# chechaohp/gan-ode

Measured on AMD Instinct MI355X. Metric: generated videos/sec (16-frame clips), higher is better.
Workload: dtype f32

## Files before the change

### gan-ode_amd/_lib.py

```python
from __future__ import annotations

import ctypes as C
import os

_HERE = os.path.dirname(os.path.abspath(__file__))
LIB_PATH = os.path.join(_HERE, "lib", "libgode.so")

i32, i64, f32, ptr = C.c_int32, C.c_int64, C.c_float, C.c_void_p
cint, u32, u64 = C.c_int, C.c_uint32, C.c_uint64

ACT_NONE, ACT_RELU, ACT_LRELU, ACT_TANH_OUT = 0, 1, 2, 3
EPI_RAW, EPI_TANH = 0, 1
FPROP, DGRAD = 0, 1
OP_IGEMM, OP_WGRAD, OP_BN_FINALIZE, OP_BN_BWD, OP_ODE_FWD, OP_ODE_BWD, OP_BCE, OP_ADAM, OP_PACK = range(1, 10)
OP_ODERNN_FWD, OP_ODERNN_BWD, OP_BN_APPLY, OP_COL2IM = 10, 11, 12, 13
OP_SDE_FWD, OP_SDE_BWD = 14, 15
OP_CDE_FWD, OP_CDE_BWD = 16, 17
OP_WGAN = 18
OP_GRU_FWD, OP_GRU_BWD = 19, 20
OP_DNOISE = 21
OP_CATEG, OP_CE = 22, 23
OP_CHSTATS, OP_CBN_EMBED, OP_CBN_EMBED_BWD, OP_CBN_APPLY, OP_CBN_BWD, OP_GRES_OUT, OP_GRES_OUT_BWD, OP_SN_FWD, OP_SN_BWD = range(24, 33)
REC_ADAM_NOISE = -1
ODE_NPARAM = 2672
# ... 111 lines not shown

class CdeFwdOp(_Op):
    _fields_ = [("p", CdeParams), ("x", ptr), ("tslope", ptr), ("content", ptr), ("sel_t", ptr), ("z", ptr),
                ("states", ptr), ("sched", ptr), ("counts", ptr), ("sync", ptr), ("N", i32), ("T", i32),
                ("S_cap", i32), ("zcols", i32), ("rtol", f32), ("atol", f32)]
    KIND, FN = OP_CDE_FWD, "gode_cde_fwd"


class CdeBwdOp(_Op):
    _fields_ = [("p", CdeParams), ("x", ptr), ("tslope", ptr), ("sel_t", ptr), ("states", ptr), ("sched", ptr),
                ("counts", ptr), ("gz", ptr), ("work", ptr), ("grads", ptr), ("N", i32), ("T", i32), ("S_cap", i32),
                ("accumulate", i32), ("zcols", i32), ("pad_", i32)]
    KIND, FN = OP_CDE_BWD, "gode_cde_bwd"


class GruParams(C.Structure):
    _fields_ = [(n, ptr) for n in "Wih Whh bih bhh".split()]


class GruFwdOp(_Op):
    _fields_ = [("p", GruParams), ("noise", ptr), ("content", ptr), ("sel_t", ptr), ("z", ptr), ("hs", ptr), ("N", i32),
                ("T", i32), ("zcols", i32), ("pad_", i32)]
    KIND, FN = OP_GRU_FWD, "gode_gru_fwd"


class GruBwdOp(_Op):
    _fields_ = [("p", GruParams), ("noise", ptr), ("hs", ptr), ("sel_t", ptr), ("gz", ptr), ("work", ptr), ("grads", ptr),
                ("N", i32), ("T", i32), ("accumulate", i32), ("zcols", i32)]
    KIND, FN = OP_GRU_BWD, "gode_gru_bwd"


class BnApplyOp(_Op):
    _fields_ = [("y", ptr), ("out", ptr), ("scale", ptr), ("shift", ptr), ("M", i64), ("C", i32), ("act", i32),
                ("M0", i64)]
    KIND, FN = OP_BN_APPLY, "gode_bn_apply"


class DnoiseOp(_Op):
    _fields_ = [("x", ptr), ("out", ptr), ("scale", ptr), ("shift", ptr), ("call_dev", ptr), ("M", i64), ("C", i32),
                ("act", i32), ("M0", i64), ("e_off", i64), ("xs", i64 * 5), ("N", i32), ("D", i32), ("H", i32), ("W", i32),
                ("seed", i64), ("stream", i32), ("layer", i32), ("call", i32), ("sigma", f32)]
    KIND, FN = OP_DNOISE, "gode_dnoise"


class Col2imOp(_Op):
    _fields_ = [("cols", ptr), ("out", ptr)] + [(n, i32) for n in "N Hi Wi Ho Wo C kh kw sh sw ph pw epilogue pad_ Di Do kd sd pd pad2_".split()]
    KIND, FN = OP_COL2IM, "gode_col2im"


class BceOp(_Op):
    _fields_ = [("logits", ptr), ("grad", ptr), ("loss", ptr), ("n", i64), ("target", f32), ("gscale", f32),
                ("accumulate", i32), ("stride", i32)]
    KIND, FN = OP_BCE, "gode_bce_logits"


class CategOp(_Op):
    _fields_ = [("cls", ptr), ("z", ptr), ("labels_out", ptr), ("n_traj", i32), ("rows_per", i32), ("C", i32),
                ("zcols", i32), ("col0", i32), ("pad_", i32)]
    KIND, FN = OP_CATEG, "gode_categ_onehot"


class CeOp(_Op):
    _fields_ = [("logits", ptr), ("labels", ptr), ("grad", ptr), ("loss", ptr), ("B", i32), ("n_lab", i32), ("C", i32),
                ("ld", i32), ("gld", i32), ("gscale", f32), ("accumulate", i32), ("rows_per_label", i32)]
    KIND, FN = OP_CE, "gode_ce_logits"


# ... 50 lines not shown
    KIND, FN = OP_SN_FWD, "gode_sn_fwd"


class SnBwdOp(_Op):
    _fields_ = [("G", ptr), ("wbar", ptr), ("u", ptr), ("v", ptr), ("sigma", ptr), ("dwbar", ptr), ("work", ptr), ("h", i32),
                ("w", i32)]
    KIND, FN = OP_SN_BWD, "gode_sn_bwd"


class AdamNoiseTensor(C.Structure):
    _fields_ = [("p", ptr), ("g", ptr), ("m", ptr), ("v", ptr), ("n", i64), ("noise_off", i64)]


class AdamOp(_Op):
    _fields_ = [("p", ptr), ("g", ptr), ("m", ptr), ("v", ptr), ("n", i64), ("lr", f32), ("beta1", f32),
                ("beta2", f32), ("eps", f32), ("weight_decay", f32), ("gscale", f32), ("step", i32), ("pad_", i32)]
    KIND, FN = OP_ADAM, "gode_adam_l2"


class PackOp(C.Structure):
    _fields_ = [("g", ConvGeom), ("dir", i32), ("co_canon", i32), ("w", ptr), ("wpack", ptr), ("co_perm", ptr)]
    KIND = OP_PACK


_OPS = _Op.__subclasses__()
_STRUCTS = {0: ConvGeom, REC_ADAM_NOISE: AdamNoiseTensor, OP_PACK: PackOp, **{st.KIND: st for st in _OPS}}

_PROTOS = {
    "gode_igemm_stats_rows": ([ptr], cint),
    "gode_igemm_stats_rows0": ([ptr], cint),
    "gode_igemm_stats_segments": ([ptr, i32, ptr], cint),
    "gode_igemm_model_cycles": ([ptr], C.c_double),
    "gode_igemm_work_size": ([ptr], i64),
    "gode_pack_size": ([ptr, cint], i64),
    "gode_pack_weights": ([ptr, cint, ptr, ptr, ptr, i32, ptr], cint),
    "gode_wgrad_work_size": ([ptr], i64),
    "gode_wgrad_auto_splits": ([ptr], cint),
    "gode_bn_bwd_work_size": ([i64, i32], i64),
    "gode_ode_bwd_work_size": ([i32], i64),
    "gode_odernn_bwd_work_size": ([i32], i64),
    "gode_odernn_sync_size": ([i32], i64),
    "gode_sde_bwd_work_size": ([i32], i64),
    "gode_cde_sync_size": ([i32], i64),
    "gode_cde_state_size": ([i32, i32], i64),
    "gode_cde_bwd_work_size": ([i32], i64),
    "gode_gru_bwd_work_size": ([i32], i64),
    "gode_ode_fwd_multi": ([ptr, i32, ptr], cint),
    "gode_ode_bwd_multi": ([ptr, i32, ptr], cint),
    "gode_odernn_fwd_multi": ([ptr, i32, ptr], cint),
    "gode_odernn_bwd_multi": ([ptr, i32, ptr], cint),
    "gode_gru_fwd_multi": ([ptr, i32, ptr], cint),
    "gode_gru_bwd_multi": ([ptr, i32, ptr], cint),
    "gode_chstats_rows": ([i64], cint),
    "gode_cbn_bwd_work_size": ([i32, i32, i32, i32], i64),
    "gode_gres_out_bwd_work_size": ([i32, i32, i32, i32, i32, i32], i64),
    "gode_scale": ([ptr, ptr, i64, f32, cint, ptr], cint),
    "gode_adam_multi": ([ptr, i32, i64, f32, f32, f32, f32, f32, f32, i32, ptr], cint),
    "gode_adam_multi_dev": ([ptr, i32, i64, f32, f32, f32, f32, f32, ptr, ptr], cint),
    "gode_adam_noise_multi": ([ptr, i32, i64, f32, f32, f32, f32, f32, f32, i32, u64, u32, u32, f32, ptr], cint),
    "gode_adam_noise_multi_dev": ([ptr, i32, i64, f32, f32, f32, f32, f32, ptr, u64, u32, f32, ptr], cint),
    "gode_param_noise": ([ptr, i64, u64, u32, u32, i64, f32, i32, ptr], cint),
    "gode_dnoise_normals": ([ptr, i64, u64, u32, u32, u32, i64, i32, ptr], cint),
    "gode_ode_step_chunks": ([ptr, i64], i64),
    "gode_ode_step": ([ptr, i32, i64, i32, f32, f32, f32, f32, f32, ptr, ptr], cint),
    "gode_axpy_multi": ([ptr, i32, i64, f32, ptr, ptr, f32, ptr, ptr, ptr], cint),
    "gode_run": ([ptr, ptr, i32, ptr], cint),
# ... 82 lines not shown
```

### gan-ode_amd/csrc/elementwise.hip

```cpp
#include "common.h"
#include "philox.h"

__global__ void __launch_bounds__(256) bn_finalize_kernel(const gode_bn_finalize_op a) {
  const int c = blockIdx.x, tid = threadIdx.x;
  __shared__ double red[2][256];
  if (a.training) {
    const int reps = a.ncols / a.C;
    const int ngroups = a.groups == 2 ? 2 : 1;
    for (int gi = 0; gi < ngroups; ++gi) {
      const int grp = ngroups == 2 ? (a.order ? 1 - gi : gi) : 0;
      double s1 = 0.0, s2 = 0.0;
      const int nseg = (ngroups == 2 && !a.stats1) ? (a.nseg > 0 ? a.nseg : 1) : 1;
      for (int sg = 0; sg < nseg; ++sg) {
        int r_lo, r_hi;
        if (ngroups == 1 || a.stats1) { r_lo = 0; r_hi = (grp == 1 && a.stats1) ? a.rows1 : a.rows; }
        else if (a.nseg > 0) { r_lo = grp == 0 ? a.seg[3 * sg] : a.seg[3 * sg + 1]; r_hi = grp == 0 ? a.seg[3 * sg + 1] : a.seg[3 * sg + 2]; }
        else { r_lo = grp == 0 ? 0 : a.rows0; r_hi = grp == 0 ? a.rows0 : a.rows; }
        const float* st = (grp == 1 && a.stats1) ? a.stats1 : a.stats;
        const int stride = (grp == 1 && a.stats1) ? a.rows1 : a.rows;
        const int nr = r_hi - r_lo;
        const int64_t items = (int64_t)nr * reps;
        for (int64_t i = tid; i < items; i += 256) {
          const int rep = (int)(i / nr); const int r = r_lo + (int)(i - (int64_t)rep * nr);
          const int64_t o = (int64_t)(rep * a.C + c) * stride + r;
          s1 += (double)st[o];
          s2 += (double)st[(int64_t)a.ncols * stride + o];
        }
      }
      __syncthreads();
      red[0][tid] = s1; red[1][tid] = s2;
      __syncthreads();
      for (int s = 128; s > 0; s >>= 1) {
        if (tid < s) { red[0][tid] += red[0][tid + s]; red[1][tid] += red[1][tid + s]; }
        __syncthreads();
      }
      if (tid == 0) {
        const double n = (double)((grp == 1 && a.count1 > 0) ? a.count1 : a.count);
        const double mean = red[0][0] / n;
        double var = red[1][0] / n - mean * mean;
        if (var < 0.0) var = 0.0;
        const float invstd = (float)(1.0 / sqrt(var + (double)a.eps));
        const float g = a.gamma ? a.gamma[c] : 1.f, b = a.beta ? a.beta[c] : 0.f;
        const float sc = g * invstd;
        const int o = grp * a.C + c;
        a.mean[o] = (float)mean; a.invstd[o] = invstd;
        a.scale[o] = sc; a.shift[o] = b - (float)mean * sc;
        if (a.running_mean) {
          const double unbiased = n > 1.0 ? var * n / (n - 1.0) : var;
          a.running_mean[c] = (1.f - a.momentum) * a.running_mean[c] + a.momentum * (float)mean;
          a.running_var[c] = (1.f - a.momentum) * a.running_var[c] + a.momentum * (float)unbiased;
        }
        if (c == 0 && a.num_batches_tracked) *a.num_batches_tracked += 1;
      }
    }
  } else if (tid == 0) {
    const float invstd = 1.f / sqrtf(a.running_var[c] + a.eps);
    const float g = a.gamma ? a.gamma[c] : 1.f, b = a.beta ? a.beta[c] : 0.f;
    const float sc = g * invstd;
    const int ngroups = a.groups == 2 ? 2 : 1;
    for (int grp = 0; grp < ngroups; ++grp) {
      const int o = grp * a.C + c;
      if (a.mean) a.mean[o] = a.running_mean[c];
      if (a.invstd) a.invstd[o] = invstd;
      a.scale[o] = sc; a.shift[o] = b - a.running_mean[c] * sc;
    }
  }
}

extern "C" int gode_bn_finalize(const gode_bn_finalize_op* op, void* stream) {
  if (!op || op->C <= 0 || !op->scale || !op->shift) return GODE_E_ARG;
  if (op->training) {
    if (!op->stats || !op->mean || !op->invstd || op->ncols % op->C != 0 || op->count <= 0) return GODE_E_ARG;
    if (op->stats1 && (op->groups != 2 || op->rows1 <= 0 || op->rows <= 0)) return GODE_E_ARG;
    if (op->groups == 2 && !op->stats1 && op->nseg == 0 && (op->rows0 <= 0 || op->rows0 >= op->rows)) return GODE_E_ARG;
    if (op->groups == 2 && (op->nseg < 0 || op->nseg > 8)) return GODE_E_ARG;
    for (int i = 0; op->groups == 2 && i < op->nseg; ++i)
      if (!(0 <= op->seg[3 * i] && op->seg[3 * i] <= op->seg[3 * i + 1] && op->seg[3 * i + 1] <= op->seg[3 * i + 2] && op->seg[3 * i + 2] <= op->rows)) return GODE_E_ARG;
  } else if (!op->running_mean || !op->running_var) return GODE_E_ARG;
  hipLaunchKernelGGL(bn_finalize_kernel, dim3(op->C), dim3(256), 0, (hipStream_t)stream, *op);
  GODE_LAUNCH_CHECK();
  return 0;
}

__global__ void __launch_bounds__(256) bn_apply_kernel(const gode_bn_apply_op a) {
  const int64_t n4 = a.M * a.C / 4;
  const float neg = a.act == GODE_ACT_RELU ? 0.f : (a.act == GODE_ACT_LRELU ? 0.2f : 1.f);
  for (int64_t i = (int64_t)blockIdx.x * 256 + threadIdx.x; i < n4; i += (int64_t)gridDim.x * 256) {
    const int c = (int)((i * 4) % a.C) + ((a.M0 > 0 && i * 4 >= a.M0 * a.C) ? a.C : 0);
    f32x4 v = *reinterpret_cast<const f32x4*>(a.y + i * 4);
    f32x4 sc = {1.f, 1.f, 1.f, 1.f}, sh = {0.f, 0.f, 0.f, 0.f};
    if (a.scale) { sc = *reinterpret_cast<const f32x4*>(a.scale + c); sh = *reinterpret_cast<const f32x4*>(a.shift + c); }
#pragma unroll
    for (int e = 0; e < 4; ++e) { const float t = v[e] * sc[e] + sh[e]; v[e] = fmaxf(t, t * neg); }
    *reinterpret_cast<f32x4*>(a.out + i * 4) = v;
  }
}

extern "C" int gode_bn_apply(const gode_bn_apply_op* op, void* stream) {
  if (!op || !op->y || !op->out || op->M <= 0 || op->C <= 0 || op->C % 4 != 0) return GODE_E_ARG;
  if ((op->scale == nullptr) != (op->shift == nullptr)) return GODE_E_ARG;
  int64_t b = (op->M * op->C / 4 + 255) / 256;
  hipLaunchKernelGGL(bn_apply_kernel, dim3((int)(b > 8192 ? 8192 : (b < 1 ? 1 : b))), dim3(256), 0, (hipStream_t)stream, *op);
  GODE_LAUNCH_CHECK();
  return 0;
}

__global__ void __launch_bounds__(256) col2im_kernel(const gode_col2im_op a) {
  const int64_t total = (int64_t)a.N * a.Ho * a.Wo;
  const int KC = a.kh * a.kw * a.C;
  for (int64_t i = (int64_t)blockIdx.x * 256 + threadIdx.x; i < total; i += (int64_t)gridDim.x * 256) {
    const int ow = (int)(i % a.Wo); const int64_t t = i / a.Wo;
    const int oh = (int)(t % a.Ho), n = (int)(t / a.Ho);
    float acc[4] = {0.f, 0.f, 0.f, 0.f};
    for (int kh = (oh + a.ph) % a.sh; kh < a.kh; kh += a.sh) {
      const int ih = (oh + a.ph - kh) / a.sh;
      if (oh + a.ph - kh < 0 || ih >= a.Hi) continue;
      for (int kw = (ow + a.pw) % a.sw; kw < a.kw; kw += a.sw) {
        const int iw = (ow + a.pw - kw) / a.sw;
        if (ow + a.pw - kw < 0 || iw >= a.Wi) continue;
        const float* src = a.cols + ((int64_t)(n * a.Hi + ih) * a.Wi + iw) * KC + (kh * a.kw + kw) * a.C;
        for (int c = 0; c < a.C; ++c) acc[c] += src[c];
      }
    }
    float* dst = a.out + i * a.C;
    for (int c = 0; c < a.C; ++c) dst[c] = a.epilogue == GODE_EPI_TANH ? tanhf(acc[c]) : acc[c];
  }
}

__global__ void __launch_bounds__(256) col2im_rows_kernel(const gode_col2im_op a, int R, int nq) {
  extern __shared__ __attribute__((aligned(16))) float c2i_lds[];
  const int KC = a.kh * a.kw * a.C, rowlen = a.Wi * KC;
  const int q = blockIdx.x % nq, n = blockIdx.x / nq;
// ... 575 lines not shown
```

### gan-ode_amd/csrc/igemm.hip

```cpp
#include <stdlib.h>
#include "common.h"
#include "conv_geom.h"

int gode_launch_conv_patch_fprop(const gode_igemm_op* op, const int64_t* gs, hipStream_t st);

struct IgemmArgs {
  IgemmGeom G;
  const float* src;
  const float* w;
  float* out;
  const float* scale;
  const float* shift;
  float* stats;
  int32_t gsN, gsD, gsH, gsW, gsC;
  int32_t act, epilogue;
  int32_t MB, NB, xcd_mode;
  int32_t tapskip, dmajor;
  int32_t stagger;
  int32_t ksplit, slabs_per_split;
  float* work;
  int32_t out_numel;
  int32_t stats_rows;
  uint32_t src_bytes, w_bytes;
};
// ... 729 lines not shown
      const float s = (part[0][threadIdx.x] + part[1][threadIdx.x]) + (part[2][threadIdx.x] + part[3][threadIdx.x]);
      a.out[oo + threadIdx.x] = a.epilogue == GODE_EPI_TANH ? tanhf(s) : s;
    }
  }
}

#define PW_MAXW 4096
struct PwArgs { IgemmArgs a; FastDiv dMw[GODE_MAX_PHASES], dMh[GODE_MAX_PHASES], dMd[GODE_MAX_PHASES]; int32_t lpp; };

template <bool ONE_TAP>
__global__ void __launch_bounds__(256) conv_pointwise_kernel(const PwArgs d) {
  const IgemmArgs& a = d.a;
  const int ph = blockIdx.y;
  const PhaseGeom& P = a.G.ph[ph];
  const int Ncols = a.G.Ncols, Cg = a.G.Cg;
  __shared__ __attribute__((aligned(16))) float wl[ONE_TAP ? 4 : PW_MAXW];
  if (!ONE_TAP) {
    for (int i = threadIdx.x; i < Ncols * P.Kp; i += 256) wl[i] = a.w[P.w_off + i];
    __syncthreads();
  }
  const int lane = threadIdx.x & 63, lpp = d.lpp, ppw = 64 / lpp;
  const int sub = lane / lpp, ch = (lane - sub * lpp) * 4;
  const float neg = a.act == GODE_ACT_RELU ? 0.f : (a.act == GODE_ACT_LRELU ? 0.2f : 1.f);
  f32x4 sc = {1.f, 1.f, 1.f, 1.f}, sh = {0.f, 0.f, 0.f, 0.f};
  if (a.scale) { sc = *reinterpret_cast<const f32x4*>(a.scale + ch); sh = *reinterpret_cast<const f32x4*>(a.shift + ch); }
  const int ntap = ONE_TAP ? 1 : P.Td * P.Th * P.Tw;
  f32x4 w1[4];
  if (ONE_TAP) {
#pragma unroll
    for (int n = 0; n < 4; ++n)
      w1[n] = n < Ncols ? *reinterpret_cast<const f32x4*>(a.w + P.w_off + (int64_t)n * P.Kp + ch) : f32x4{0.f, 0.f, 0.f, 0.f};
  }
  const int64_t wave_id = (int64_t)blockIdx.x * 4 + (threadIdx.x >> 6), nwaves = (int64_t)gridDim.x * 4;
  for (int64_t m0 = wave_id * ppw; m0 < P.M; m0 += nwaves * ppw) {
    const int m = (int)m0 + sub;
    const bool live = m < P.M;
    const uint32_t mm = live ? (uint32_t)m : 0u;
    const uint32_t t1 = fdiv(mm, d.dMw[ph]), qw = mm - t1 * P.Mw;
    const uint32_t t2 = fdiv(t1, d.dMh[ph]), qh = t1 - t2 * P.Mh;
    const uint32_t img = fdiv(t2, d.dMd[ph]), qd = t2 - img * P.Md;
    const int bd = (int)qd * a.G.Sd + P.Od, bh = (int)qh * a.G.Sh + P.Oh, bw = (int)qw * a.G.Sw + P.Ow;
    const int base = (int)img * a.gsN;
    float acc[4] = {0.f, 0.f, 0.f, 0.f};
    int jd = 0, jh = 0, jw = 0;
    for (int t = 0; t < ntap; ++t) {
      const int id = bd + a.G.J * jd, ih = bh + a.G.J * jh, iw = bw + a.G.J * jw;
      const bool ok = live && (unsigned)id < (unsigned)a.G.Gd && (unsigned)ih < (unsigned)a.G.Gh && (unsigned)iw < (unsigned)a.G.Gw;
      if (ok) {
        f32x4 v = *reinterpret_cast<const f32x4*>(a.src + base + id * a.gsD + ih * a.gsH + iw * a.gsW + ch);
#pragma unroll
        for (int e = 0; e < 4; ++e) { const float u = v[e] * sc[e] + sh[e]; v[e] = fmaxf(u, u * neg); }
        const float* wk = wl + t * Cg + ch;
#pragma unroll
        for (int n = 0; n < 4; ++n)
          if (ONE_TAP || n < Ncols) {
            const f32x4 w = ONE_TAP ? w1[n] : *reinterpret_cast<const f32x4*>(wk + n * P.Kp);
            acc[n] += v[0] * w[0] + v[1] * w[1] + v[2] * w[2] + v[3] * w[3];
          }
      }
      if (++jw == P.Tw) { jw = 0; if (++jh == P.Th) { jh = 0; ++jd; } }
    }
    for (int o = lpp >> 1; o > 0; o >>= 1) {
#pragma unroll
      for (int n = 0; n < 4; ++n) acc[n] += __shfl_xor(acc[n], o);
    }
    if (live && ch == 0) {
// ... 625 lines not shown
```

### gan-ode_amd/engine.py

```python
from __future__ import annotations

import ctypes as C
from dataclasses import dataclass
from typing import List, Optional, Sequence

import numpy as np
import torch

from . import _lib as L


def make_geom(N, Ci, Co, xi, yo, k, s, p) -> L.ConvGeom:
    return L.ConvGeom(N, Ci, Co, xi[0], xi[1], xi[2], yo[0], yo[1], yo[2], k[0], k[1], k[2], s[0], s[1], s[2],
                      p[0], p[1], p[2])


def conv_out(i, k, s, p):
    return (i + 2 * p - k) // s + 1


def dptr(t: Optional[torch.Tensor]):
    return None if t is None else t.data_ptr()


# ... 31 lines not shown
    beta: Optional[torch.Tensor] = None
    running_mean: Optional[torch.Tensor] = None
    running_var: Optional[torch.Tensor] = None
    num_batches_tracked: Optional[torch.Tensor] = None


def _contig_strides(dims):
    n, d, h, w, c = dims
    return (d * h * w * c, h * w * c, w * c, c, 1)


class ConvStack:

    def __init__(self, specs: Sequence[LayerSpec], params: Sequence[LayerParams], device, owns_input: bool,
                 momentum=0.1, eps=1e-5, pack_cache: Optional[dict] = None, groups: int = 1, split_images: int = 0,
                 split_order: int = 0, two_lane_backward: bool = False):
        self.specs, self.params, self.device = list(specs), list(params), device
        self.groups = groups
        self.two_lane = bool(two_lane_backward)
        self._lane_stream = None
        self.split, self.split_order = int(split_images), int(split_order)
        if self.split and (groups != 1 or not owns_input or not (0 < self.split < specs[0].geom.N)):
            raise ValueError("split ConvStack: plan-owned input, one launch group, 0 < split_images < N")
        self._G2 = groups == 2 or self.split > 0
        self._last_parts = False
        if groups not in (1, 2) or (groups == 2 and (owns_input or specs[0].fwd_dir != L.FPROP or specs[0].has_bn
                                                     or specs[0].geom.N % 2)):
            raise ValueError("grouped ConvStack: two groups, Conv stack, caller-owned input, no BatchNorm on layer 0")
        self.nl = len(specs)
        self.noisy = any(s.noise for s in specs)
        if self.noisy and (owns_input or self.split):
            raise ValueError("instance noise: caller-owned input, no split stack")
        self.momentum, self.eps = momentum, eps
        self.busy = False
        self.generation = 0
        self._fwd_training = True
        self.pack_cache = pack_cache if pack_cache is not None else {}
        lib = L.lib()
        f32 = dict(dtype=torch.float32, device=device)
        self.x_in = torch.zeros(specs[0].in_dims(), **f32) if owns_input else None
        self.x0n = torch.empty(specs[0].in_dims(), **f32) if specs[0].noise else None
        self.y = [torch.empty(s.out_dims(), **f32) for s in specs[:-1]]
        self.a = [torch.empty(s.out_dims(), **f32) if self._materialize(l) else None for l, s in enumerate(specs[:-1])]
        self.out_dims = specs[-1].out_dims()
        self.wpack_f, self.wpack_b = [], [None] * self.nl
        self.stats, self.stat_rows = [], []
        self.mean, self.invstd, self.scale, self.shift = [], [], [], []
        self._two_f, self._two_b, self._rows_ab = {}, {}, {}
        for l, s in enumerate(specs):
            n = lib.gode_pack_size(C.byref(s.geom), s.fwd_dir)
            if n <= 0:
                raise RuntimeError(f"bad geometry for pack ({n})")
            self.wpack_f.append(self._shared_pack(l, s.fwd_dir, n))
            C_out = s.out_dims()[4]
            two = self._two_f[l] = bool(self.split) and 0 < l < self.nl - 1 and self._two_launches(s.geom, s.fwd_dir)
            if s.has_bn:
                probe = L.IgemmOp(g=s.geom, dir=s.fwd_dir, tile=0, groups=groups)
                if two:
                    ra, rb = (lib.gode_igemm_stats_rows(C.byref(L.IgemmOp(g=self._part_geom(s.geom, n), dir=s.fwd_dir, tile=0)))
                              for n in (self.split, s.geom.N - self.split))
                    rows = ra + rb if ra > 0 and rb > 0 else -1
                    self._rows_ab[l] = (ra, rb)
                else:
                    rows = lib.gode_igemm_stats_rows(C.byref(probe))
                if rows <= 0:
                    raise RuntimeError(f"layer {l}: no partial-statistics layout for this geometry ({rows})")
# ... 228 lines not shown
                    raise RuntimeError("a one-layer stack cannot use the GEMM + col2im head")
                continue
            want_stats = s.has_bn and training
            if self._last_parts and l == self.nl - 1:
                per_in, per_out, Cs = int(np.prod(s.in_dims()[1:])), int(np.prod(s.out_dims()[1:])), sc.numel() // 2
                pair = []
                for n, img0, k in ((self.split, 0, 0), (s.geom.N - self.split, self.split, 1)):
                    pair.append(L.IgemmOp(g=self._part_geom(s.geom, n), dir=s.fwd_dir, act=act, epilogue=s.epilogue, tile=0,
                                          src=src.data_ptr() + 4 * img0 * per_in, wpack=dptr(self.wpack_f[l]), out=None,
                                          scale=sc.data_ptr() + 4 * Cs * k, shift=sh.data_ptr() + 4 * Cs * k))
                ops += pair
                patch["last"], patch["last2"] = pair[0], (pair[1], 4 * self.split * per_out)
                continue
            if self._two_f.get(l):
                ra = self._rows_ab[l][0] if s.has_bn else 0
                per_in, per_out = int(np.prod(s.in_dims()[1:])), int(np.prod(s.out_dims()[1:]))
                for n, img0, st_off in ((self.split, 0, 0), (s.geom.N - self.split, self.split, ra * 2 * self._ncols(s))):
                    ops.append(L.IgemmOp(g=self._part_geom(s.geom, n), dir=s.fwd_dir, act=act, epilogue=s.epilogue, tile=0,
                                         src=src.data_ptr() + 4 * img0 * per_in, wpack=dptr(self.wpack_f[l]),
                                         out=self.y[l].data_ptr() + 4 * img0 * per_out, scale=dptr(sc), shift=dptr(sh),
                                         stats=self.stats[l].data_ptr() + 4 * st_off if want_stats else None, groups=0))
                op = None
            else:
                op = L.IgemmOp(g=s.geom, dir=s.fwd_dir, act=act, epilogue=s.epilogue, tile=0, src=dptr(src),
                               wpack=dptr(self.wpack_f[l]), out=dptr(self.y[l]) if l < self.nl - 1 else None,
                               scale=dptr(sc), shift=dptr(sh),
                               stats=dptr(self.stats[l]) if want_stats else None,
                               groups=2 if (G2 and s.has_bn) else 0)
                ops.append(op)
            if l == 0:
                patch["first"] = op
            if l == self.nl - 1:
                patch["last"] = op
            if s.has_bn:
                rows0 = lib.gode_igemm_stats_rows0(C.byref(op)) if G2 else 0
                fin = L.BnFinalizeOp(stats=dptr(self.stats[l]), rows=self.stat_rows[l], ncols=self._ncols(s),
                                     C=s.out_dims()[4], count=self._count(l) // self.groups, gamma=dptr(p.gamma),
                                     beta=dptr(p.beta), running_mean=dptr(p.running_mean),
                                     running_var=dptr(p.running_var),
                                     num_batches_tracked=dptr(p.num_batches_tracked), mean=dptr(self.mean[l]),
                                     invstd=dptr(self.invstd[l]), scale=dptr(self.scale[l]),
                                     shift=dptr(self.shift[l]), momentum=self.momentum, eps=self.eps,
                                     training=1 if training else 0, groups=self.groups if G2 else 0, rows0=rows0)
                if self.split:
                    per_img = self._count(l) // s.geom.N
                    fin.groups, fin.order = 2, self.split_order
                    fin.count, fin.count1 = per_img * self.split, per_img * (s.geom.N - self.split)
                    if self._two_f.get(l):
                        ra, rb = self._rows_ab[l]
                        fin.rows, fin.rows1 = ra, rb
                        fin.stats1 = self.stats[l].data_ptr() + 4 * ra * 2 * self._ncols(s)
                    else:
                        nseg, seg = self._segs[l]
                        fin.nseg = nseg
                        for k in range(3 * nseg):
                            fin.seg[k] = seg[k]
                ops.append(fin)
            if l < self.nl - 1 and self.a[l] is not None:
                d = s.out_dims()
                M = d[0] * d[1] * d[2] * d[3]
                M0 = M // 2 if (G2 and s.has_bn) else ((M // d[0]) * self.split if (self.split and s.has_bn) else 0)
                if self.specs[l + 1].noise:
                    ops.append(self._noise_op(noise, l, dptr(self.scale[l]), dptr(self.shift[l]), M // 2 if G2 else 0))
                    continue
                ops.append(L.BnApplyOp(y=dptr(self.y[l]), out=dptr(self.a[l]), scale=dptr(self.scale[l]),
                                       shift=dptr(self.shift[l]), M=M, C=d[4], act=s.act, M0=M0))
        patch["packs"] = packs
        self._attach_work([op for op in ops if isinstance(op, L.IgemmOp)])
        return L.Program(ops), patch

    def _noise_op(self, noise, l, scale, shift, M0):
        d = self.specs[l].out_dims()
        op = L.DnoiseOp(x=dptr(self.y[l]), out=dptr(self.a[l]), scale=scale, shift=shift, M=d[0] * d[1] * d[2] * d[3],
                        C=d[4], act=self.specs[l].act, M0=M0, layer=l + 1)
        noise.append((op, d[1] * d[2] * d[3] * d[4], 0, None))
        return op

    @staticmethod
    def _patch_noise(patch, noise, inputs):
        seed = int(noise["seed"]) & 0xFFFFFFFFFFFFFFFF
        seed = seed - (1 << 64) if seed >= 1 << 63 else seed
        dev = noise.get("call_dev")
        base = 0 if dev else int(noise["call"])
        for op, per, add, k in patch["noise"]:
            op.seed, op.stream, op.sigma = seed, int(noise["stream"]), float(noise["sigma"])
            c = (base + add) & 0xFFFFFFFF
            op.call_dev, op.call = dev, c - (1 << 32) if c >= 1 << 31 else c
            op.e_off = int(noise.get("sample_offset", 0)) * per
            if k is not None:
                x, xs = inputs[k]
                op.x = x.data_ptr()
                for i in range(5):
                    op.xs[i] = int(xs[i])

    def forward(self, training: bool, x: Optional[torch.Tensor] = None, x_strides=None, pre_ops_program=None,
                x2: Optional[torch.Tensor] = None, x2_strides=None, noise=None):
        self._refresh()
        if training not in self._fwd:
            self._fwd[training] = self._build_fwd(training)
        prog, patch = self._fwd[training]
        if self.noisy:
            if noise is None:
# ... 285 lines not shown
```

### include/gode.h

```cpp
#ifndef GODE_H
#define GODE_H
#include <stdint.h>
#ifdef __cplusplus
extern "C" {
#endif

#define GODE_VERSION 105

enum { GODE_OK = 0, GODE_E_ARG = -1, GODE_E_SHAPE = -2, GODE_E_KIND = -3 };
enum { GODE_ACT_NONE = 0, GODE_ACT_RELU = 1, GODE_ACT_LRELU = 2,
       GODE_ACT_TANH_OUT = 3  };
enum { GODE_EPI_RAW = 0, GODE_EPI_TANH = 1 };
enum { GODE_FPROP = 0, GODE_DGRAD = 1 };

typedef struct gode_conv_geom {
  int32_t N, Ci, Co;
  int32_t Di, Hi, Wi;
  int32_t Do, Ho, Wo;
  int32_t kd, kh, kw;
  int32_t sd, sh, sw;
  int32_t pd, ph, pw;
} gode_conv_geom;

typedef struct gode_igemm_op {
// ... 20 lines not shown
                      int32_t co_canon, void* stream);

typedef struct gode_wgrad_op {
  gode_conv_geom g;
  int32_t act, xform_on_y, splits, accumulate;
  const float* x;
  const float* y;
  const float* scale;
  const float* shift;
  float* work;
  float* dw;
  const int32_t* co_perm; int64_t co_canon;
  int64_t xs[5];
} gode_wgrad_op;
int gode_wgrad(const gode_wgrad_op* op, void* stream);
int64_t gode_wgrad_work_size(const gode_wgrad_op* op);
int gode_wgrad_auto_splits(const gode_conv_geom* g);

typedef struct gode_bn_finalize_op {
  const float* stats; int32_t rows, ncols, C; int64_t count;
  const float* gamma; const float* beta;
  float* running_mean; float* running_var; int64_t* num_batches_tracked;
  float* mean; float* invstd; float* scale; float* shift;
  float momentum, eps; int32_t training, pad_;
  int32_t groups, rows0;
  int32_t nseg, order; int64_t count1; int32_t seg[24];
  const float* stats1; int32_t rows1, pad3_;
} gode_bn_finalize_op;
int gode_bn_finalize(const gode_bn_finalize_op* op, void* stream);

typedef struct gode_bn_apply_op {
  const float* y; float* out; const float* scale; const float* shift; int64_t M; int32_t C, act;
  int64_t M0;
} gode_bn_apply_op;
int gode_bn_apply(const gode_bn_apply_op* op, void* stream);

typedef struct gode_col2im_op {
  const float* cols; float* out;
  int32_t N, Hi, Wi, Ho, Wo, C, kh, kw, sh, sw, ph, pw;
  int32_t epilogue, pad_;
  int32_t Di, Do, kd, sd, pd, pad2_;
} gode_col2im_op;
int gode_col2im(const gode_col2im_op* op, void* stream);

typedef struct gode_bn_bwd_op {
  float* g; const float* y; int64_t M; int32_t C, act;
  const float* gamma; const float* mean; const float* invstd; const float* scale; const float* shift;
  float* dgamma; float* dbeta; float* work; int32_t accumulate, eval_mode;
  const float* gin;
  int32_t groups, pad2_;
  int64_t M0;
  const float* r1_s; const float* r1_w; int32_t r1_H, r1_W, r1_h, r1_wd, r1_off, pad3_;
} gode_bn_bwd_op;
int gode_bn_bwd(const gode_bn_bwd_op* op, void* stream);
int64_t gode_bn_bwd_work_size(int64_t M, int32_t C);

typedef struct gode_ode_params {
  const float* Wa; const float* ba; const float* Wb; const float* bb;
  const float* W1; const float* b1; const float* W2; const float* b2;
} gode_ode_params;
typedef struct gode_ode_fwd_op {
  gode_ode_params p;
  const float* x; const float* content; const float* dt; const int32_t* sel_t;
  float* z; float* traj; int32_t N, T, substeps, prenet;
  int32_t zcols, G;
  const float* grid_dt; const int32_t* emit_at; const float* emit_w;
  int32_t method, pad2_; float rtol, atol; const float* tout; int32_t* nsteps;
  int32_t* sync;
// ... 285 lines not shown
```

Measured before the change: 35290.

## Fold BN finalize into BN apply kernel and unroll one-tap pointwise path

Adds a fused bn_apply_fold kernel. Each block recomputes the per-channel batch-norm statistics for a slice of channels, then applies scale, shift and activation to a chunk of rows. This removes a separate finalize launch and its dependency. The price is redundant re-reading of the stats across row chunks, and a cost model decides when the fold is used. A separate change adds a 4-way unrolled one-tap path in the igemm pointwise kernel to batch its loads.

New measurement: 34050. 3.5% lower.

```diff
diff --git a/gan-ode_amd/_lib.py b/gan-ode_amd/_lib.py
--- a/gan-ode_amd/_lib.py
+++ b/gan-ode_amd/_lib.py
@@ -167,7 +167,7 @@
 
 class BnApplyOp(_Op):
     _fields_ = [("y", ptr), ("out", ptr), ("scale", ptr), ("shift", ptr), ("M", i64), ("C", i32), ("act", i32),
-                ("M0", i64)]
+                ("M0", i64), ("fold", i32), ("pad_", i32), ("fin", BnFinalizeOp)]
     KIND, FN = OP_BN_APPLY, "gode_bn_apply"
 
 
@@ -284,6 +284,7 @@
     "gode_igemm_stats_segments": ([ptr, i32, ptr], cint),
     "gode_igemm_model_cycles": ([ptr], C.c_double),
     "gode_igemm_work_size": ([ptr], i64),
+    "gode_bn_apply_fold_pays": ([i32, i32, i32, i64], cint),
     "gode_pack_size": ([ptr, cint], i64),
     "gode_pack_weights": ([ptr, cint, ptr, ptr, ptr, i32, ptr], cint),
     "gode_wgrad_work_size": ([ptr], i64),
diff --git a/gan-ode_amd/csrc/elementwise.hip b/gan-ode_amd/csrc/elementwise.hip
--- a/gan-ode_amd/csrc/elementwise.hip
+++ b/gan-ode_amd/csrc/elementwise.hip
@@ -1,32 +1,87 @@
 #include "common.h"
 #include "philox.h"
+
+
+__device__ __forceinline__ int bn_ngroups(const gode_bn_finalize_op& a) { return a.groups == 2 ? 2 : 1; }
+__device__ __forceinline__ int bn_group(const gode_bn_finalize_op& a, int gi) { return a.groups == 2 ? (a.order ? 1 - gi : gi) : 0; }
+
+struct BnSeg { const float* st; int64_t plane; int stride, r_lo, nr, reps; int64_t items; };
+__device__ __forceinline__ int64_t bn_item(const gode_bn_finalize_op& a, const BnSeg& s, int c, int64_t i) {
+  const int rep = (int)(i / s.nr); const int r = s.r_lo + (int)(i - (int64_t)rep * s.nr);
+  return (int64_t)(rep * a.C + c) * s.stride + r;
+}
+template <class F>
+__device__ __forceinline__ void bn_walk(const gode_bn_finalize_op& a, int grp, F&& f) {
+  const int ngroups = bn_ngroups(a);
+  const int nseg = (ngroups == 2 && !a.stats1) ? (a.nseg > 0 ? a.nseg : 1) : 1;
+  for (int sg = 0; sg < nseg; ++sg) {
+    int r_lo, r_hi;
+    if (ngroups == 1 || a.stats1) { r_lo = 0; r_hi = (grp == 1 && a.stats1) ? a.rows1 : a.rows; }
+    else if (a.nseg > 0) { r_lo = grp == 0 ? a.seg[3 * sg] : a.seg[3 * sg + 1]; r_hi = grp == 0 ? a.seg[3 * sg + 1] : a.seg[3 * sg + 2]; }
+    else { r_lo = grp == 0 ? 0 : a.rows0; r_hi = grp == 0 ? a.rows0 : a.rows; }
+    BnSeg s;
+    s.st = (grp == 1 && a.stats1) ? a.stats1 : a.stats;
+    s.stride = (grp == 1 && a.stats1) ? a.rows1 : a.rows;
+    s.plane = (int64_t)a.ncols * s.stride;
+    s.r_lo = r_lo; s.nr = r_hi - r_lo; s.reps = a.ncols / a.C;
+    s.items = (int64_t)s.nr * s.reps;
+    f(s);
+  }
+}
+__device__ __forceinline__ void bn_channel_train(const gode_bn_finalize_op& a, int c, int grp, double s1, double s2, bool write,
+                                                 float& sc_out, float& sh_out) {
+  const double n = (double)((grp == 1 && a.count1 > 0) ? a.count1 : a.count);
+  const double mean = s1 / n;
+  double var = s2 / n - mean * mean;
+  if (var < 0.0) var = 0.0;
+  const float invstd = (float)(1.0 / sqrt(var + (double)a.eps));
+  const float g = a.gamma ? a.gamma[c] : 1.f, b = a.beta ? a.beta[c] : 0.f;
+  const float sc = g * invstd;
+  const float sh = b - (float)mean * sc;
+  sc_out = sc; sh_out = sh;
+  if (write) {
+    const int o = grp * a.C + c;
+    a.mean[o] = (float)mean; a.invstd[o] = invstd;
+    a.scale[o] = sc; a.shift[o] = sh;
+    if (a.running_mean) {
+      const double unbiased = n > 1.0 ? var * n / (n - 1.0) : var;
+      a.running_mean[c] = (1.f - a.momentum) * a.running_mean[c] + a.momentum * (float)mean;
+      a.running_var[c] = (1.f - a.momentum) * a.running_var[c] + a.momentum * (float)unbiased;
+    }
+    if (c == 0 && a.num_batches_tracked) *a.num_batches_tracked += 1;
+  }
+}
+__device__ __forceinline__ void bn_channel_eval(const gode_bn_finalize_op& a, int c, bool write, float& sc_out, float& sh_out) {
+  const float invstd = 1.f / sqrtf(a.running_var[c] + a.eps);
+  const float g = a.gamma ? a.gamma[c] : 1.f, b = a.beta ? a.beta[c] : 0.f;
+  const float sc = g * invstd;
+  const float sh = b - a.running_mean[c] * sc;
+  sc_out = sc; sh_out = sh;
+  if (write) {
+    for (int grp = 0; grp < bn_ngroups(a); ++grp) {
+      const int o = grp * a.C + c;
+      if (a.mean) a.mean[o] = a.running_mean[c];
+      if (a.invstd) a.invstd[o] = invstd;
+      a.scale[o] = sc; a.shift[o] = sh;
+    }
+  }
+}
 
 __global__ void __launch_bounds__(256) bn_finalize_kernel(const gode_bn_finalize_op a) {
   const int c = blockIdx.x, tid = threadIdx.x;
   __shared__ double red[2][256];
+  float sc, sh;
   if (a.training) {
-    const int reps = a.ncols / a.C;
-    const int ngroups = a.groups == 2 ? 2 : 1;
-    for (int gi = 0; gi < ngroups; ++gi) {
-      const int grp = ngroups == 2 ? (a.order ? 1 - gi : gi) : 0;
+    for (int gi = 0; gi < bn_ngroups(a); ++gi) {
+      const int grp = bn_group(a, gi);
       double s1 = 0.0, s2 = 0.0;
-      const int nseg = (ngroups == 2 && !a.stats1) ? (a.nseg > 0 ? a.nseg : 1) : 1;
-      for (int sg = 0; sg < nseg; ++sg) {
-        int r_lo, r_hi;
-        if (ngroups == 1 || a.stats1) { r_lo = 0; r_hi = (grp == 1 && a.stats1) ? a.rows1 : a.rows; }
-        else if (a.nseg > 0) { r_lo = grp == 0 ? a.seg[3 * sg] : a.seg[3 * sg + 1]; r_hi = grp == 0 ? a.seg[3 * sg + 1] : a.seg[3 * sg + 2]; }
-        else { r_lo = grp == 0 ? 0 : a.rows0; r_hi = grp == 0 ? a.rows0 : a.rows; }
-        const float* st = (grp == 1 && a.stats1) ? a.stats1 : a.stats;
-        const int stride = (grp == 1 && a.stats1) ? a.rows1 : a.rows;
-        const int nr = r_hi - r_lo;
-        const int64_t items = (int64_t)nr * reps;
-        for (int64_t i = tid; i < items; i += 256) {
-          const int rep = (int)(i / nr); const int r = r_lo + (int)(i - (int64_t)rep * nr);
-          const int64_t o = (int64_t)(rep * a.C + c) * stride + r;
-          s1 += (double)st[o];
-          s2 += (double)st[(int64_t)a.ncols * stride + o];
+      bn_walk(a, grp, [&](const BnSeg& s) {
+        for (int64_t i = tid; i < s.items; i += 256) {
+          const int64_t o = bn_item(a, s, c, i);
+          s1 += (double)s.st[o];
+          s2 += (double)s.st[s.plane + o];
         }
-      }
+      });
       __syncthreads();
       red[0][tid] = s1; red[1][tid] = s2;
       __syncthreads();
@@ -34,40 +89,12 @@
         if (tid < s) { red[0][tid] += red[0][tid + s]; red[1][tid] += red[1][tid + s]; }
         __syncthreads();
       }
-      if (tid == 0) {
-        const double n = (double)((grp == 1 && a.count1 > 0) ? a.count1 : a.count);
-        const double mean = red[0][0] / n;
-        double var = red[1][0] / n - mean * mean;
-        if (var < 0.0) var = 0.0;
-        const float invstd = (float)(1.0 / sqrt(var + (double)a.eps));
-        const float g = a.gamma ? a.gamma[c] : 1.f, b = a.beta ? a.beta[c] : 0.f;
-        const float sc = g * invstd;
-        const int o = grp * a.C + c;
-        a.mean[o] = (float)mean; a.invstd[o] = invstd;
-        a.scale[o] = sc; a.shift[o] = b - (float)mean * sc;
-        if (a.running_mean) {
-          const double unbiased = n > 1.0 ? var * n / (n - 1.0) : var;
-          a.running_mean[c] = (1.f - a.momentum) * a.running_mean[c] + a.momentum * (float)mean;
-          a.running_var[c] = (1.f - a.momentum) * a.running_var[c] + a.momentum * (float)unbiased;
-        }
-        if (c == 0 && a.num_batches_tracked) *a.num_batches_tracked += 1;
-      }
-    }
-  } else if (tid == 0) {
-    const float invstd = 1.f / sqrtf(a.running_var[c] + a.eps);
-    const float g = a.gamma ? a.gamma[c] : 1.f, b = a.beta ? a.beta[c] : 0.f;
-    const float sc = g * invstd;
-    const int ngroups = a.groups == 2 ? 2 : 1;
-    for (int grp = 0; grp < ngroups; ++grp) {
-      const int o = grp * a.C + c;
-      if (a.mean) a.mean[o] = a.running_mean[c];
-      if (a.invstd) a.invstd[o] = invstd;
-      a.scale[o] = sc; a.shift[o] = b - a.running_mean[c] * sc;
-    }
-  }
-}
-
-extern "C" int gode_bn_finalize(const gode_bn_finalize_op* op, void* stream) {
+      if (tid == 0) bn_channel_train(a, c, grp, red[0][0], red[1][0], true, sc, sh);
+    }
+  } else if (tid == 0) bn_channel_eval(a, c, true, sc, sh);
+}
+
+static int bn_finalize_check(const gode_bn_finalize_op* op) {
   if (!op || op->C <= 0 || !op->scale || !op->shift) return GODE_E_ARG;
   if (op->training) {
     if (!op->stats || !op->mean || !op->invstd || op->ncols % op->C != 0 || op->count <= 0) return GODE_E_ARG;
@@ -77,27 +104,178 @@
     for (int i = 0; op->groups == 2 && i < op->nseg; ++i)
       if (!(0 <= op->seg[3 * i] && op->seg[3 * i] <= op->seg[3 * i + 1] && op->seg[3 * i + 1] <= op->seg[3 * i + 2] && op->seg[3 * i + 2] <= op->rows)) return GODE_E_ARG;
   } else if (!op->running_mean || !op->running_var) return GODE_E_ARG;
+  return 0;
+}
+
+extern "C" int gode_bn_finalize(const gode_bn_finalize_op* op, void* stream) {
+  const int rc = bn_finalize_check(op);
+  if (rc) return rc;
   hipLaunchKernelGGL(bn_finalize_kernel, dim3(op->C), dim3(256), 0, (hipStream_t)stream, *op);
   GODE_LAUNCH_CHECK();
   return 0;
 }
+
+__device__ __forceinline__ f32x4 bn_act4(f32x4 v, const f32x4& sc, const f32x4& sh, float neg) {
+#pragma unroll
+  for (int e = 0; e < 4; ++e) { const float t = v[e] * sc[e] + sh[e]; v[e] = fmaxf(t, t * neg); }
+  return v;
+}
+__device__ __forceinline__ float bn_neg_slope(int act) { return act == GODE_ACT_RELU ? 0.f : (act == GODE_ACT_LRELU ? 0.2f : 1.f); }
 
 __global__ void __launch_bounds__(256) bn_apply_kernel(const gode_bn_apply_op a) {
   const int64_t n4 = a.M * a.C / 4;
-  const float neg = a.act == GODE_ACT_RELU ? 0.f : (a.act == GODE_ACT_LRELU ? 0.2f : 1.f);
+  const float neg = bn_neg_slope(a.act);
   for (int64_t i = (int64_t)blockIdx.x * 256 + threadIdx.x; i < n4; i += (int64_t)gridDim.x * 256) {
     const int c = (int)((i * 4) % a.C) + ((a.M0 > 0 && i * 4 >= a.M0 * a.C) ? a.C : 0);
-    f32x4 v = *reinterpret_cast<const f32x4*>(a.y + i * 4);
+    const f32x4 v = *reinterpret_cast<const f32x4*>(a.y + i * 4);
     f32x4 sc = {1.f, 1.f, 1.f, 1.f}, sh = {0.f, 0.f, 0.f, 0.f};
     if (a.scale) { sc = *reinterpret_cast<const f32x4*>(a.scale + c); sh = *reinterpret_cast<const f32x4*>(a.shift + c); }
-#pragma unroll
-    for (int e = 0; e < 4; ++e) { const float t = v[e] * sc[e] + sh[e]; v[e] = fmaxf(t, t * neg); }
-    *reinterpret_cast<f32x4*>(a.out + i * 4) = v;
-  }
+    *reinterpret_cast<f32x4*>(a.out + i * 4) = bn_act4(v, sc, sh, neg);
+  }
+}
+
+#ifndef BN_FOLD_SLICE
+#define BN_FOLD_SLICE 32
+#endif
+#define BN_FOLD_WGS 512
+struct BnFoldGrid { int32_t nslices, nchunks; int64_t rows_per_chunk; };
+
+__device__ __forceinline__ double bn_fold_sum(const gode_bn_finalize_op& f, int grp, int which, int c, int j) {
+  double acc[32];
+#pragma unroll
+  for (int k = 0; k < 32; ++k) acc[k] = 0.0;
+  bn_walk(f, grp, [&](const BnSeg& s) {
+    const float* st = s.st + (int64_t)which * s.plane;
+    int64_t base = 0;
+    for (; base + 256 <= s.items; base += 256) {
+      float v[32];
+#pragma unroll
+      for (int k = 0; k < 32; ++k) {
+        const int64_t i = base + 8 * k + j;
+        v[k] = st[s.reps == 1 ? (int64_t)c * s.stride + s.r_lo + i : bn_item(f, s, c, i)];
+      }
+#pragma unroll
+      for (int k = 0; k < 32; ++k) acc[k] += (double)v[k];
+    }
+    if (base < s.items) {
+#pragma unroll
+      for (int kb = 0; kb < 32; kb += 8) {
+        if (base + 8 * kb < s.items) {
+          float v[8];
+#pragma unroll
+          for (int k = 0; k < 8; ++k) {
+            const int64_t i = base + 8 * (kb + k) + j;
+            const bool ok = i < s.items;
+            const int64_t o = s.reps == 1 ? (int64_t)c * s.stride + s.r_lo + (ok ? i : 0) : bn_item(f, s, c, ok ? i : 0);
+            const float x = st[o];
+            v[k] = ok ? x : 0.f;
+          }
+#pragma unroll
+          for (int k = 0; k < 8; ++k) acc[kb + k] += (double)v[k];
+        }
+      }
+    }
+  });
+#pragma unroll
+  for (int s = 16; s > 0; s >>= 1) {
+#pragma unroll
+    for (int k = 0; k < 16; ++k)
+      if (k < s) acc[k] += acc[k + s];
+  }
+  double x = acc[0];
+#pragma unroll
+  for (int s = 4; s > 0; s >>= 1) x += __shfl_xor(x, s);
+  return x;
+}
+
+__global__ void __launch_bounds__(256) bn_apply_fold_kernel(const gode_bn_apply_op a, const BnFoldGrid g) {
+  const gode_bn_finalize_op& f = a.fin;
+  __shared__ __attribute__((aligned(16))) float ssc[2][BN_FOLD_SLICE], ssh[2][BN_FOLD_SLICE];
+  const int tid = threadIdx.x;
+  const int sl = (int)(blockIdx.x % g.nslices), chunk = (int)(blockIdx.x / g.nslices);
+  const int c0 = sl * BN_FOLD_SLICE;
+  const bool writer = chunk == 0;
+  for (int cb = 0; cb < BN_FOLD_SLICE; cb += 32) {
+    const int cl = cb + (tid >> 3), c = c0 + cl, j = tid & 7;
+    const bool live = c < f.C;
+    const int cc = live ? c : 0;
+    float sc = 1.f, sh = 0.f;
+    if (f.training) {
+      for (int gi = 0; gi < bn_ngroups(f); ++gi) {
+        const int grp = bn_group(f, gi);
+        const double s1 = bn_fold_sum(f, grp, 0, cc, j);
+        const double s2 = bn_fold_sum(f, grp, 1, cc, j);
+        if (live) {
+          bn_channel_train(f, c, grp, s1, s2, writer && j == 0, sc, sh);
+          if (j == 0) { ssc[grp][cl] = sc; ssh[grp][cl] = sh; }
+        }
+      }
+    } else if (live && j == 0) {
+      bn_channel_eval(f, c, writer, sc, sh);
+      ssc[0][cl] = sc; ssh[0][cl] = sh; ssc[1][cl] = sc; ssh[1][cl] = sh;
+    }
+  }
+  __syncthreads();
+  constexpr int LPR = BN_FOLD_SLICE / 4, RPI = 256 / LPR;
+  const int q = tid % LPR, c = c0 + q * 4;
+  if (c >= a.C) return;
+  const float neg = bn_neg_slope(a.act);
+  const f32x4 sc0 = *reinterpret_cast<const f32x4*>(&ssc[0][q * 4]), sh0 = *reinterpret_cast<const f32x4*>(&ssh[0][q * 4]);
+  const f32x4 sc1 = *reinterpret_cast<const f32x4*>(&ssc[1][q * 4]), sh1 = *reinterpret_cast<const f32x4*>(&ssh[1][q * 4]);
+  const int64_t m_lo = chunk * g.rows_per_chunk;
+  const int64_t m_hi = m_lo + g.rows_per_chunk < a.M ? m_lo + g.rows_per_chunk : a.M;
+  for (int64_t m = m_lo + tid / LPR; m < m_hi; m += 4 * RPI) {
+    f32x4 v[4];
+#pragma unroll
+    for (int u = 0; u < 4; ++u)
+      if (m + u * RPI < m_hi) v[u] = *reinterpret_cast<const f32x4*>(a.y + (m + u * RPI) * a.C + c);
+#pragma unroll
+    for (int u = 0; u < 4; ++u)
+      if (m + u * RPI < m_hi) {
+        const bool second = a.M0 > 0 && m + u * RPI >= a.M0;
+        *reinterpret_cast<f32x4*>(a.out + (m + u * RPI) * a.C + c) = bn_act4(v[u], second ? sc1 : sc0, second ? sh1 : sh0, neg);
+      }
+  }
+}
+
+static int bn_fold_grid(const gode_bn_apply_op* op, BnFoldGrid* g) {
+  const int64_t nsl = (op->C + BN_FOLD_SLICE - 1) / BN_FOLD_SLICE;
+  int64_t nch = (BN_FOLD_WGS + nsl - 1) / nsl;
+  const int64_t rpi = 256 / (BN_FOLD_SLICE / 4);
+  if (nch > (op->M + rpi - 1) / rpi) nch = (op->M + rpi - 1) / rpi;
+  if (nch < 1) nch = 1;
+  g->nslices = (int32_t)nsl;
+  g->rows_per_chunk = (op->M + nch - 1) / nch;
+  g->nchunks = (int32_t)((op->M + g->rows_per_chunk - 1) / g->rows_per_chunk);
+  return nsl * g->nchunks < (1ll << 31) ? 0 : GODE_E_SHAPE;
+}
+
+#define BN_FOLD_MAX_REREAD 0.5
+extern "C" int gode_bn_apply_fold_pays(int32_t rows, int32_t ncols, int32_t C, int64_t M) {
+  if (rows <= 0 || C <= 0 || C % 4 != 0 || ncols <= 0 || ncols % C != 0 || M <= 0) return GODE_E_ARG;
+  gode_bn_apply_op op = {};
+  op.C = C; op.M = M;
+  BnFoldGrid g;
+  if (bn_fold_grid(&op, &g)) return 0;
+  const double reread = (double)g.nslices * g.nchunks * BN_FOLD_SLICE * ((double)rows * (ncols / C)) * 8.0;
+  const double pass = (double)M * C * 8.0;
+  return reread <= BN_FOLD_MAX_REREAD * pass ? 1 : 0;
 }
 
 extern "C" int gode_bn_apply(const gode_bn_apply_op* op, void* stream) {
   if (!op || !op->y || !op->out || op->M <= 0 || op->C <= 0 || op->C % 4 != 0) return GODE_E_ARG;
+  if (op->fold) {
+    const int rc = bn_finalize_check(&op->fin);
+    if (rc) return rc;
+    if (op->fin.C != op->C) return GODE_E_ARG;
+    if (op->fin.training && (int64_t)(op->fin.rows > op->fin.rows1 ? op->fin.rows : op->fin.rows1) * (op->fin.ncols / op->fin.C) >= (1ll << 31))
+      return GODE_E_SHAPE;
+    BnFoldGrid g;
+    if (bn_fold_grid(op, &g)) return GODE_E_SHAPE;
+    hipLaunchKernelGGL(bn_apply_fold_kernel, dim3(g.nslices * g.nchunks), dim3(256), 0, (hipStream_t)stream, *op, g);
+    GODE_LAUNCH_CHECK();
+    return 0;
+  }
   if ((op->scale == nullptr) != (op->shift == nullptr)) return GODE_E_ARG;
   int64_t b = (op->M * op->C / 4 + 255) / 256;
   hipLaunchKernelGGL(bn_apply_kernel, dim3((int)(b > 8192 ? 8192 : (b < 1 ? 1 : b))), dim3(256), 0, (hipStream_t)stream, *op);
diff --git a/gan-ode_amd/csrc/igemm.hip b/gan-ode_amd/csrc/igemm.hip
--- a/gan-ode_amd/csrc/igemm.hip
+++ b/gan-ode_amd/csrc/igemm.hip
@@ -785,6 +785,48 @@
       w1[n] = n < Ncols ? *reinterpret_cast<const f32x4*>(a.w + P.w_off + (int64_t)n * P.Kp + ch) : f32x4{0.f, 0.f, 0.f, 0.f};
   }
   const int64_t wave_id = (int64_t)blockIdx.x * 4 + (threadIdx.x >> 6), nwaves = (int64_t)gridDim.x * 4;
+  if (ONE_TAP) {
+    constexpr int PW_U = 4;
+    for (int64_t m0 = wave_id * (PW_U * ppw); m0 < P.M; m0 += nwaves * (PW_U * ppw)) {
+      const int m = (int)m0 + sub;
+      const uint32_t mm = m < P.M ? (uint32_t)m : 0u;
+      const uint32_t t1 = fdiv(mm, d.dMw[ph]), t2 = fdiv(t1, d.dMh[ph]);
+      int qw = (int)(mm - t1 * P.Mw), qh = (int)(t1 - t2 * P.Mh), img = (int)fdiv(t2, d.dMd[ph]), qd = (int)t2 - img * P.Md;
+      f32x4 v[PW_U]; bool ok[PW_U]; int oo[PW_U];
+#pragma unroll
+      for (int u = 0; u < PW_U; ++u) {
+        const int id = qd * a.G.Sd + P.Od, ih = qh * a.G.Sh + P.Oh, iw = qw * a.G.Sw + P.Ow;
+        ok[u] = m + u * ppw < P.M && (unsigned)id < (unsigned)a.G.Gd && (unsigned)ih < (unsigned)a.G.Gh && (unsigned)iw < (unsigned)a.G.Gw;
+        const int off = ok[u] ? img * a.gsN + id * a.gsD + ih * a.gsH + iw * a.gsW : 0;
+        v[u] = *reinterpret_cast<const f32x4*>(a.src + off + ch);
+        oo[u] = m + u * ppw < P.M ? (((img * a.G.Xd + qd * a.G.OSd + P.Pd) * a.G.Xh + qh * a.G.OSh + P.Ph) * a.G.Xw + qw * a.G.OSw + P.Pw) * Ncols : -1;
+        qw += ppw;
+        while (qw >= P.Mw) { qw -= P.Mw; if (++qh == P.Mh) { qh = 0; if (++qd == P.Md) { qd = 0; ++img; } } }
+      }
+#pragma unroll
+      for (int u = 0; u < PW_U; ++u) {
+        float acc[4] = {0.f, 0.f, 0.f, 0.f};
+        f32x4 x = v[u];
+#pragma unroll
+        for (int e = 0; e < 4; ++e) { const float t = x[e] * sc[e] + sh[e]; x[e] = fmaxf(t, t * neg); }
+#pragma unroll
+        for (int n = 0; n < 4; ++n)
+          if (n < Ncols) {
+            acc[n] += x[0] * w1[n][0] + x[1] * w1[n][1] + x[2] * w1[n][2] + x[3] * w1[n][3];
+            if (!ok[u]) acc[n] = 0.f;
+          }
+        for (int o = lpp >> 1; o > 0; o >>= 1) {
+#pragma unroll
+          for (int n = 0; n < 4; ++n)
+            if (n < Ncols) acc[n] += __shfl_xor(acc[n], o);
+        }
+        if (oo[u] >= 0 && ch == 0) {
+          for (int n = 0; n < Ncols; ++n) a.out[oo[u] + n] = a.epilogue == GODE_EPI_TANH ? tanhf(acc[n]) : acc[n];
+        }
+      }
+    }
+    return;
+  }
   for (int64_t m0 = wave_id * ppw; m0 < P.M; m0 += nwaves * ppw) {
     const int m = (int)m0 + sub;
     const bool live = m < P.M;
diff --git a/gan-ode_amd/engine.py b/gan-ode_amd/engine.py
--- a/gan-ode_amd/engine.py
+++ b/gan-ode_amd/engine.py
@@ -87,6 +87,7 @@
         if self.noisy and (owns_input or self.split):
             raise ValueError("instance noise: caller-owned input, no split stack")
         self.momentum, self.eps = momentum, eps
+        self.fold_bn = None
         self.busy = False
         self.generation = 0
         self._fwd_training = True
@@ -381,6 +382,7 @@
                 patch["first"] = op
             if l == self.nl - 1:
                 patch["last"] = op
+            fin = None
             if s.has_bn:
                 rows0 = lib.gode_igemm_stats_rows0(C.byref(op)) if G2 else 0
                 fin = L.BnFinalizeOp(stats=dptr(self.stats[l]), rows=self.stat_rows[l], ncols=self._ncols(s),
@@ -404,19 +406,33 @@
                         fin.nseg = nseg
                         for k in range(3 * nseg):
                             fin.seg[k] = seg[k]
-                ops.append(fin)
             if l < self.nl - 1 and self.a[l] is not None:
                 d = s.out_dims()
                 M = d[0] * d[1] * d[2] * d[3]
                 M0 = M // 2 if (G2 and s.has_bn) else ((M // d[0]) * self.split if (self.split and s.has_bn) else 0)
                 if self.specs[l + 1].noise:
+                    if fin is not None:
+                        ops.append(fin)
                     ops.append(self._noise_op(noise, l, dptr(self.scale[l]), dptr(self.shift[l]), M // 2 if G2 else 0))
                     continue
-                ops.append(L.BnApplyOp(y=dptr(self.y[l]), out=dptr(self.a[l]), scale=dptr(self.scale[l]),
-                                       shift=dptr(self.shift[l]), M=M, C=d[4], act=s.act, M0=M0))
+                app = L.BnApplyOp(y=dptr(self.y[l]), out=dptr(self.a[l]), scale=dptr(self.scale[l]),
+                                  shift=dptr(self.shift[l]), M=M, C=d[4], act=s.act, M0=M0)
+                if fin is not None and self._fold(fin, M):
+                    app.fold, app.fin = 1, fin
+                elif fin is not None:
+                    ops.append(fin)
+                ops.append(app)
+            elif fin is not None:
+                ops.append(fin)
         patch["packs"] = packs
         self._attach_work([op for op in ops if isinstance(op, L.IgemmOp)])
         return L.Program(ops), patch
+
+    def _fold(self, fin, M):
+        if self.fold_bn is not None:
+            return bool(self.fold_bn)
+        rows = max(fin.rows, fin.rows1)
+        return L.lib().gode_bn_apply_fold_pays(rows, fin.ncols, fin.C, M) == 1
 
     def _noise_op(self, noise, l, scale, shift, M0):
         d = self.specs[l].out_dims()
diff --git a/include/gode.h b/include/gode.h
--- a/include/gode.h
+++ b/include/gode.h
@@ -76,8 +76,10 @@
 typedef struct gode_bn_apply_op {
   const float* y; float* out; const float* scale; const float* shift; int64_t M; int32_t C, act;
   int64_t M0;
+  int32_t fold, pad_; gode_bn_finalize_op fin;
 } gode_bn_apply_op;
 int gode_bn_apply(const gode_bn_apply_op* op, void* stream);
+int gode_bn_apply_fold_pays(int32_t rows, int32_t ncols, int32_t C, int64_t M);
 
 typedef struct gode_col2im_op {
   const float* cols; float* out;
```
